# smpurkis/PyTorch-Face-Detection-from-Scratch

Hardware: AMD Instinct MI355X
Metric: train imgs/sec (PoolResnet 480^2, bs=256 per GPU) (higher is better)
Workload: dtype f32 (3x3 convs: bf16x3 split MFMA, fp32 accumulate)

## Files before the change

### pytorch-face-detection-from-scratch_amd/csrc/fdet_conv3x3_ps.hip

```cpp
#include "fdet_conv3x3_x3.h"
#include "fdet_ps.h"
#include "fdet_ldsdma.h"
#include <algorithm>

using namespace fdet;

typedef __attribute__((address_space(3))) void* lds_void_t;
typedef const __attribute__((address_space(1))) void* glb_void_t;
typedef unsigned u32x4 __attribute__((ext_vector_type(4)));

namespace {

#ifndef PS_DBG
#define PS_DBG 0
#endif
constexpr int PSA = 9 * 2 * 64;
constexpr int PS_ROWI = 10;

enum { PSE_FWD_FULL = 0, PSE_DGRAD_ACT = 1, PSE_FWD_POOL = 2, PSE_DGRAD_ADDPOOL = 3 };

struct PsConvArgs {
  const bf16x8* x;
  const bf16x8* a_hi;
  const bf16x8* a_lo;
// ... 22 lines not shown
__device__ __forceinline__ void ps_keep(const f32x16& v) {
#if defined(__HIP_DEVICE_COMPILE__)
  asm volatile("" ::"v"(v));
#endif
}

__device__ __forceinline__ void ps_opaque(unsigned& v) {
#if defined(__HIP_DEVICE_COMPILE__)
  asm("" : "+v"(v));
#endif
}

__device__ __forceinline__ int ps_lane_now() {
  int v = 0;
#if defined(__HIP_DEVICE_COMPILE__)
  asm volatile("v_mbcnt_lo_u32_b32 %0, -1, 0\n\tv_mbcnt_hi_u32_b32 %0, -1, %0" : "=v"(v));
#endif
  return v;
}

__device__ __forceinline__ void ps_acc_read(const f32x16& acc, const int r, float& z) {
#if defined(__HIP_DEVICE_COMPILE__)
  asm("v_accvgpr_read_b32 %0, %1" : "=v"(z) : "a"(acc[r]));
#else
  z = acc[r];
#endif
}

template <int MODE, bool P16>
__device__ __forceinline__ void ps_unit(const f32x16& acc, const int gp, const float (&bza)[4], const float (&bzb)[4],
                                        const u32x2_t (&sg)[2], const float slope, const bool ok, const int ob, const int m,
                                        const int half, const int gstride, const int plane_o_bytes,
                                        const __amdgpu_buffer_rsrc_t yrs) {
  float za[4], zb[4];
#pragma unroll
  for (int i = 0; i < 4; ++i) {
#if defined(__HIP_DEVICE_COMPILE__)
    asm("v_accvgpr_read_b32 %0, %1" : "=v"(za[i]) : "a"(acc[8 * gp + i]));
    asm("v_accvgpr_read_b32 %0, %1" : "=v"(zb[i]) : "a"(acc[8 * gp + 4 + i]));
#else
    za[i] = acc[8 * gp + i]; zb[i] = acc[8 * gp + 4 + i];
#endif
  }
  if (MODE == PSE_FWD_FULL) {
#pragma unroll
    for (int i = 0; i < 4; ++i) {
      const float wa = za[i] + bza[i], wb = zb[i] + bzb[i];
      za[i] = fmaxf(wa, wa * slope);
      zb[i] = fmaxf(wb, wb * slope);
    }
  } else if (MODE == PSE_DGRAD_ACT) {
#pragma unroll
    for (int i = 0; i < 4; ++i) {
      za[i] *= ps_join(sg[0][i >> 1], 0u, i & 1) > 0.f ? 1.f : slope;
      zb[i] *= ps_join(sg[1][i >> 1], 0u, i & 1) > 0.f ? 1.f : slope;
    }
  }
  unsigned ha[2], la[2], hb[2], lb[2];
  if (P16) {
    ps_hi4(za, ha);
    ps_hi4(zb, hb);
  } else {
    ps_split4(za, ha, la);
    ps_split4(zb, hb, lb);
  }
#pragma unroll
  for (int k = 0; k < 2; ++k) {
    auto r1 = __builtin_amdgcn_permlane32_swap(ha[k], hb[k], false, false);
    ha[k] = r1[0]; hb[k] = r1[1];
    if (!P16) {
      auto r2 = __builtin_amdgcn_permlane32_swap(la[k], lb[k], false, false);
      la[k] = r2[0]; lb[k] = r2[1];
    }
  }
  const int G = 4 * m + 2 * gp + half;
  const unsigned off = ok ? (unsigned)(ob + G * gstride) * 16u : 0x80000000u;
  __builtin_amdgcn_raw_buffer_store_b128(u32x4{ha[0], ha[1], hb[0], hb[1]}, yrs, off, 0, 0);
  if (!P16) __builtin_amdgcn_raw_buffer_store_b128(u32x4{la[0], la[1], lb[0], lb[1]}, yrs, off, plane_o_bytes, 0);
}

template <int MODE, int WP, bool P16, bool WG2 = false>
__global__ void __launch_bounds__(256, WG2 ? 2 : 1)
k_conv3x3_ps(const PsConvArgs p) {
  static_assert(!WG2 || MODE == PSE_FWD_POOL, "two workgroups per CU: the pooled forward only (one accumulator set)");
  constexpr bool WOVEN = MODE == PSE_FWD_FULL || MODE == PSE_DGRAD_ACT || MODE == PSE_DGRAD_ADDPOOL;
  extern __shared__ __attribute__((aligned(16))) char smem[];
  bf16x8* const lds = reinterpret_cast<bf16x8*>(smem);
  const int tid = threadIdx.x, lane = tid & 63;
  const int wid = __builtin_amdgcn_readfirstlane(tid >> 6);
  const int l31 = lane & 31, half = lane >> 5;
  constexpr int WPL = WP == 64 ? 6 : 5, R = 512 / WP, PT = (R + 2) * WP + 8, NBI = (R + 2) * WP / 64;
  constexpr int buf_units = 2 * PSA + 4 * PT;
  const int HP = p.HP;
  int qn[4];
#pragma unroll
  for (int n = 0; n < 4; ++n) qn[n] = WP == 64 ? (2 * wid + (n & 1)) * 64 + (n >> 1) * 32 : (4 * wid + n) * 32;
  constexpr bool POOLM = MODE == PSE_FWD_POOL || MODE == PSE_DGRAD_ADDPOOL;
  if (POOLM) {
#pragma unroll
    for (int n = 0; n < 4; ++n) qn[n] = (WP == 64 ? (2 * wid + (n >> 1)) * 64 : (4 * wid + (n >> 1)) * 32) + (n & 1);
  }
  const int lb = POOLM ? (WP == 64 ? 2 * l31 : 2 * l31 + 32 * (l31 >> 4)) : l31;
  int tile = blockIdx.x, tend = p.ntiles, tstep = gridDim.x;
  if ((gridDim.x & 7) == 0) {
    const int grp = blockIdx.x & 7, chunk = (p.ntiles + 7) >> 3;
    tile = grp * chunk + (blockIdx.x >> 3);
    tend = min((grp + 1) * chunk, p.ntiles);
    tstep = gridDim.x >> 3;
    if (tile >= tend) tile = tend = p.ntiles;
  }
  if (tile >= tend) return;

  unsigned ro[PS_ROWI];
#define PS_ROWOFF(T)                                                                               \
  {                                                                                                \
    const int v0_ = (T) * R;                                                                       \
    _Pragma("unroll") for (int i_ = 0; i_ < PS_ROWI; ++i_) {                                       \
      const int u_ = i_ * 64 + lane;                                                               \
      const int vv_ = v0_ - 1 + (u_ >> WPL) + HP;                                                  \
      const int nn_ = (int)__umulhi((unsigned)vv_, p.magic_hp);                                    \
      ro[i_] = (unsigned)(((PS_DBG & 8) ? 1 : nn_) * p.img_i + (vv_ - nn_ * HP) * WP + (u_ & (WP - 1))) * 16u; \
    }                                                                                              \
  }
  const unsigned lds0 = (unsigned)(size_t)(lds_void_t)smem;
  const dma_u32x4 wrs = dma_rsrc((wid >> 1) ? p.a_lo : p.a_hi, (unsigned)p.nch * PSA * 16u);
  const dma_u32x4 xrs = dma_rsrc(p.x - p.img_i, (unsigned)(p.N + 2) * (unsigned)p.img_i * 16u);
  const unsigned wvoff = (unsigned)((wid & 1) * 576 + lane) * 16u;
#define PS_DMA(C, BS)                                                                              \
  if (!(PS_DBG & 4) && !(P16 && wid >= 2)) {                  \
    const unsigned db_ = lds0 + (unsigned)(BS) * (buf_units * 16);                                 \
    const unsigned ad_ = db_ + (unsigned)((wid >> 1) * PSA + (wid & 1) * 576) * 16u;               \
    _Pragma("unroll") for (int k_ = 0; k_ < ((PS_DBG & 16) ? 0 : 9); ++k_)                          \
      dma_piece(ad_ + k_ * 1024, wvoff, wrs, (unsigned)(C) * (PSA * 16) + k_ * 1024);              \
    const unsigned bso_ = (unsigned)((wid >> 1) * p.plane_i + (2 * (C) + (wid & 1)) * HP * WP) * 16u; \
    const unsigned bd_ = db_ + (unsigned)(2 * PSA + wid * PT) * 16u;                               \
    _Pragma("unroll") for (int i_ = 0; i_ < NBI; ++i_) dma_piece(bd_ + i_ * 1024, ro[i_], xrs, bso_); \
  }

  f32x16 accA[2][4], accB[WOVEN ? 2 : 1][WOVEN ? 4 : 1];
  if (WOVEN) {
#pragma unroll
    for (int m = 0; m < 2; ++m)
#pragma unroll
      for (int n = 0; n < 4; ++n)
#pragma unroll
        for (int r = 0; r < 16; ++r) accB[WOVEN ? m : 0][WOVEN ? n : 0][r] = 0.f;
  }

  float bz[2][4][4];
#pragma unroll
  for (int m = 0; m < 2; ++m)
#pragma unroll
    for (int g = 0; g < 4; ++g)
#pragma unroll
      for (int i = 0; i < 4; ++i) bz[m][g][i] = ((MODE == PSE_FWD_FULL || MODE == PSE_FWD_POOL) && !WG2) ? p.bias[32 * m + 8 * g + 4 * half + i] : 0.f;

  const int a_off = half * 64 + l31;
  const int b_off = 2 * PSA + half * PT + lb;
  const int gstride = HP * WP, plane_o_bytes = p.plane_o * 16;
  const __amdgpu_buffer_rsrc_t yrs = __builtin_amdgcn_make_buffer_rsrc(p.y, 0, (int)((size_t)p.N * p.img_o * 16), 0x00020000);

  int ob[4];
  bool okn[4];
#pragma unroll
  for (int n = 0; n < 4; ++n) { ob[n] = 0; okn[n] = false; }
#define PS_GEO(T)                                                                                  \
  {                                                                                                \
    _Pragma("unroll") for (int n_ = 0; n_ < 4; ++n_) {                                             \
// ... 95 lines not shown
    }                                                                                              \
    _Pragma("unroll") for (int n_ = 0; n_ < 4; ++n_) {                                             \
      bh[F][n_] = Bw[qn[n_] + to_];                                                                \
      if (!P16) bl[F][n_] = Bw[2 * PT + qn[n_] + to_];                                             \
    }                                                                                              \
  }
#define PS_BODY(ACC, FIRST, JOB, PREV)                                                             \
  {                                                                                                \
    const bf16x8* buf_ = lds + sb * buf_units;                                                     \
    const bf16x8* Aw = buf_ + a_off;                                                               \
    const bf16x8* Bw = buf_ + b_off;                                                               \
    PS_FRAGS(0, 0)                                                                                 \
    __builtin_amdgcn_sched_barrier(0);                                                             \
    _Pragma("unroll") for (int t = 0; t < 9; ++t) {                                                \
      const int F = t & 1;                                                                         \
      if (t < 8) PS_FRAGS(F ^ 1, t + 1)                                                            \
      if (!(PS_DBG & 2)) {                                                                         \
        _Pragma("unroll") for (int m = 0; m < 2; ++m)                                              \
          _Pragma("unroll") for (int n = 0; n < 4; ++n) {                                          \
            const f32x16 zero_ = {};                                                               \
            if (P16) {                                                                             \
              ACC[m][n] = __builtin_amdgcn_mfma_f32_32x32x16_bf16(ah[F][m], bh[F][n], ((FIRST) && t == 0) ? zero_ : ACC[m][n], 0, 0, 0); \
            } else {                                                                               \
              ACC[m][n] = __builtin_amdgcn_mfma_f32_32x32x16_bf16(ah[F][m], bl[F][n], ((FIRST) && t == 0) ? zero_ : ACC[m][n], 0, 0, 0); \
              ACC[m][n] = __builtin_amdgcn_mfma_f32_32x32x16_bf16(al[F][m], bh[F][n], ACC[m][n], 0, 0, 0); \
              ACC[m][n] = __builtin_amdgcn_mfma_f32_32x32x16_bf16(ah[F][m], bh[F][n], ACC[m][n], 0, 0, 0); \
            }                                                                                      \
          }                                                                                        \
      }                                                                                            \
      if ((JOB) != 0 && t < 8 && !(PS_DBG & 1)) {                                                  \
        if constexpr (MODE == PSE_DGRAD_ADDPOOL) {                                                 \
           \
          _Pragma("unroll") for (int e_ = 0; e_ < 2; ++e_) {                                       \
            const int it_ = ((JOB) - 1) * 16 + 2 * t + e_;                                         \
            const int m_ = it_ >> 4, gp_ = (it_ >> 3) & 1, ab_ = (it_ >> 2) & 1, i_ = it_ & 3;     \
            const int arg_ = (int)((rkp[m_][gp_][ab_] >> (8 * i_ + 4)) & 3u);                      \
            const float gv_ = dgp[m_][gp_][ab_][i_];                                               \
            const int so_ = (32 * m_ + 16 * gp_ + 8 * ab_ + i_) * p.H * p.Wf * 4;                  \
            _Pragma("unroll") for (int r_ = 0; r_ < 2; ++r_) {                                     \
              float z0_, z1_;                                                                      \
              ps_acc_read(PREV[WOVEN ? m_ : 0][WOVEN ? 2 * r_ : 0], 8 * gp_ + 4 * ab_ + i_, z0_);  \
              ps_acc_read(PREV[WOVEN ? m_ : 0][WOVEN ? 2 * r_ + 1 : 0], 8 * gp_ + 4 * ab_ + i_, z1_); \
              z0_ += arg_ == 2 * r_ ? gv_ : 0.f;                                                   \
              z1_ += arg_ == 2 * r_ + 1 ? gv_ : 0.f;                                               \
              __builtin_amdgcn_raw_buffer_store_b64(u32x2_t{__builtin_bit_cast(unsigned, z0_), __builtin_bit_cast(unsigned, z1_)}, prs, sto, \
                                                    so_ + r_ * p.Wf * 4, 0);                       \
            }                                                                                      \
          }                                                                                        \
        } else {                                                                                   \
          const int n_ = ((JOB) - 1) * 2 + (t >> 2), m_ = (t >> 1) & 1, gp_ = t & 1;               \
          ps_unit<MODE, P16>(PREV[WOVEN ? m_ : 0][WOVEN ? n_ : 0], gp_, bz[m_][2 * gp_], bz[m_][2 * gp_ + 1], sgp[n_][m_][gp_], p.slope, okn[n_], ob[n_], m_, \
                        half, gstride, plane_o_bytes, yrs);                                        \
        }                                                                                          \
      }                                                                                            \
       \
       \
      if (P16) {    \
        _Pragma("unroll") for (int i = 0; i < 8; ++i) {                                            \
          __builtin_amdgcn_sched_group_barrier(0x008, 1, 0);                                       \
          if (i < 6) __builtin_amdgcn_sched_group_barrier(0x100, 1, 0);                            \
          if ((JOB) != 0) __builtin_amdgcn_sched_group_barrier(0x002, 6, 0);                       \
          if ((JOB) != 0 && (i >= 7 || (MODE == PSE_DGRAD_ADDPOOL && i >= 4))) __builtin_amdgcn_sched_group_barrier(0x040, 1, 0); \
        }                                                                                          \
      } else {                                                                                     \
      _Pragma("unroll") for (int i = 0; i < 12; ++i) {                                             \
        __builtin_amdgcn_sched_group_barrier(0x008, 1, 0);                                         \
        __builtin_amdgcn_sched_group_barrier(0x100, 1, 0);                                         \
        if ((JOB) != 0) __builtin_amdgcn_sched_group_barrier(0x002, 3, 0);                         \
      }                                                                                            \
      _Pragma("unroll") for (int i = 0; i < 12; ++i) {                                             \
        __builtin_amdgcn_sched_group_barrier(0x008, 1, 0);                                         \
        if ((JOB) != 0) __builtin_amdgcn_sched_group_barrier(0x002, 3, 0);                         \
        if ((JOB) != 0 && (i >= 10 || (MODE == PSE_DGRAD_ADDPOOL && i >= 8))) __builtin_amdgcn_sched_group_barrier(0x040, 1, 0); \
      }                                                                                            \
      }                                                                                            \
    }                                                                                              \
    sb ^= 1;                                                                                       \
  }
  const __amdgpu_buffer_rsrc_t prs = __builtin_amdgcn_make_buffer_rsrc(MODE == PSE_FWD_POOL ? (void*)p.pool_ps : (void*)p.dx_f32, 0,
      MODE == PSE_FWD_POOL ? (int)((size_t)p.N * p.img_p * 16) : (int)((size_t)p.Nimg * 64 * p.H * p.Wf * 4), 0x00020000);
  const __amdgpu_buffer_rsrc_t frs = __builtin_amdgcn_make_buffer_rsrc(p.pool_f32, 0, (int)((size_t)p.Nimg * 64 * p.Hp * p.Wpf * 4), 0x00020000);
  const __amdgpu_buffer_rsrc_t rrs = __builtin_amdgcn_make_buffer_rsrc(p.route_out, 0, (int)((size_t)p.N * 64 * p.Hp * p.Wp), 0x00020000);
  const __amdgpu_buffer_rsrc_t srs = __builtin_amdgcn_make_buffer_rsrc((void*)p.scale, 0, (WG2 && p.scale) ? (int)((size_t)p.Nimg * 64 * 4) : 0, 0x00020000);
  const __amdgpu_buffer_rsrc_t ars = __builtin_amdgcn_make_buffer_rsrc((void*)p.aux, 0, WG2 ? (int)((size_t)p.N * p.img_i * 16) : 0, 0x00020000);
  const __amdgpu_buffer_rsrc_t brs = __builtin_amdgcn_make_buffer_rsrc((void*)p.bias, 0, (WG2 && p.bias) ? 64 * 4 : 0, 0x00020000);
  const int pool_cnt = MODE == PSE_FWD_POOL ? 4 * ((P16 ? 1 : 2) * (p.pool_ps != nullptr) + (p.route_out != nullptr) + 8 * (p.pool_f32 != nullptr)) : 63;
#define PS_WIN(T)                                                                                  \
    const int rb_ = WP == 64 ? 2 * wid : 4 * wid + 2 * (l31 >> 4);                                 \
    const int v_ = (T) * R + rb_;                                                                  \
    const int nn = (int)__umulhi((unsigned)v_, p.magic_hp), y = v_ - nn * HP;                      \
    const int xp = WP == 64 ? l31 : (l31 & 15), yp = y >> 1;                                       \
    const bool okw = nn < p.N && y < p.H && 2 * xp < (nn >= p.last0 ? p.Wlast : p.W);              \
                \
    const int si = p.last0 == 0 ? 0 : (p.Nimg == 1 ? nn : (int)__umulhi((unsigned)nn, p.magic_nimg)); \
    const int ni = nn - si * p.Nimg, xg = si * (p.xo >> 1) + xp;
  float dgp[2][2][2][4];
  unsigned rkp[2][2][2];
  unsigned sto = 0x80000000u;
#pragma unroll
  for (int m = 0; m < 2; ++m)
#pragma unroll
    for (int gp = 0; gp < 2; ++gp)
#pragma unroll
      for (int ab = 0; ab < 2; ++ab) {
        rkp[m][gp][ab] = 0u;
#pragma unroll
        for (int i = 0; i < 4; ++i) dgp[m][gp][ab][i] = 0.f;
      }
#define PS_POOLPREF(T)                                                                             \
  {                                                                                                \
    PS_WIN(T)                                                                                      \
    const int HWp = p.Hp * p.Wpf, HWr = p.Hp * p.Wp;                                               \
    const int pbase = okw ? (ni * 64 * p.Hp + yp) * p.Wpf + xg : 0;                                \
    const int rbase = okw ? (nn * 8 * p.Hp + yp) * p.Wp + xp : 0;                                  \
    _Pragma("unroll") for (int m = 0; m < 2; ++m)                                                  \
      _Pragma("unroll") for (int gp = 0; gp < 2; ++gp)                                             \
        _Pragma("unroll") for (int ab = 0; ab < 2; ++ab) {                                         \
          const int G = 4 * m + 2 * gp + ab;                                                       \
          _Pragma("unroll") for (int i = 0; i < 4; ++i) {                                          \
            const float v_ = p.dout[pbase + (8 * G + 4 * half + i) * HWp];                         \
            dgp[m][gp][ab][i] = okw ? v_ : 0.f;                                                    \
          }                                                                                        \
          rkp[m][gp][ab] = *reinterpret_cast<const unsigned*>(p.route_in + (size_t)(rbase + G * HWr) * 8 + 4 * half); \
        }                                                                                          \
    sto = okw ? (unsigned)(((ni * 64 + 4 * half) * p.H + y) * p.Wf + 2 * xg) * 4u : 0x80000000u;   \
  }
#define PS_EPI_LOADS(M, GP)                                                                        \
  {                                                                                                \
    const size_t ga = (size_t)(4 * (M) + 2 * (GP)) * gstride, gb = ga + (size_t)gstride;           \
    _Pragma("unroll") for (int n = 0; n < 4; ++n) {                                                \
      const u32x2_t* ap = reinterpret_cast<const u32x2_t*>(p.aux + sb0 + (n >> 1) * WP + (n & 1)) + half; \
      sk[M][GP][n][0] = ap[ga * 2];                                                                \
      sk[M][GP][n][1] = P16 ? u32x2_t{0u, 0u} : ap[(ga + p.plane_i) * 2];                          \
      sk[M][GP][n][2] = ap[gb * 2];                                                                \
      sk[M][GP][n][3] = P16 ? u32x2_t{0u, 0u} : ap[(gb + p.plane_i) * 2];                          \
    }                                                                                              \
    _Pragma("unroll") for (int i = 0; i < 4; ++i) {                                                \
      const int ch = 32 * (M) + 16 * (GP) + 4 * half + i;                                          \
      scv[M][GP][0][i] = (p.scale && okw) ? p.scale[ni * 64 + ch] : 1.f;                           \
      scv[M][GP][1][i] = (p.scale && okw) ? p.scale[ni * 64 + ch + 8] : 1.f;                       \
      bzw[M][2 * (GP)][i] = bz[M][2 * (GP)][i];                                                    \
      bzw[M][2 * (GP) + 1][i] = bz[M][2 * (GP) + 1][i];                                            \
    }                                                                                              \
  }
#define PS_EPI_LOADS_G(M, GP, AB)                                                                  \
  {                                                                                                \
    const int g_ = (4 * (M) + 2 * (GP) + (AB)) * gstride * 16;                                     \
    _Pragma("unroll") for (int n = 0; n < 4; ++n) {    \
      const int n_ = ((n >> 1) * WP + (n & 1)) * 16;                                               \
      sk[M][GP][n][2 * (AB)] = __builtin_amdgcn_raw_buffer_load_b64(ars, skoff, g_ + n_, 0);       \
      sk[M][GP][n][2 * (AB) + 1] = P16 ? u32x2_t{0u, 0u} : __builtin_amdgcn_raw_buffer_load_b64(ars, skoff, g_ + p.plane_i * 16 + n_, 0); \
    }                                                                                              \
    _Pragma("unroll") for (int i = 0; i < 4; ++i) {                                                \
      const int ch = 32 * (M) + 16 * (GP) + 8 * (AB) + i;                                          \
      const unsigned sv_ = __builtin_amdgcn_raw_buffer_load_b32(srs, scoff, ch * 4, 0);            \
      scv[M][GP][AB][i] = __uint_as_float((sv_ & scm) | (0x3f800000u & ~scm));    \
      bzw[M][2 * (GP) + (AB)][i] = __uint_as_float(__builtin_amdgcn_raw_buffer_load_b32(brs, (unsigned)halfe * 16u, ch * 4, 0)); \
    }                                                                                              \
  }
#define PS_EPI_ST_F32(M, GP)                                                                       \
  {                                                                                                \
    const unsigned off = okw ? (unsigned)(((ni * 64 + 32 * (M) + 16 * (GP) + 4 * halfe) * p.Hp + yp) * p.Wpf + xg) * 4u : 0x80000000u;\
    _Pragma("unroll") for (int jj = 0; jj < 8; ++jj)                                               \
      __builtin_amdgcn_raw_buffer_store_b32(__builtin_bit_cast(unsigned, pvs[M][GP][jj >> 2][jj & 3]), frs, off,\
                                            (8 * (jj >> 2) + (jj & 3)) * p.Hp * p.Wpf * 4, 0);     \
  }
#define PS_EPI_XCHG(M, GP)                                                                         \
// ... 62 lines not shown
          }                                                                                        \
          _Pragma("unroll") for (int i = 0; i < 4; ++i) {                                          \
            float mx = -INFINITY;                                                                  \
            int arg = 0;                                                                           \
            unsigned bits = 0;                                                                     \
            _Pragma("unroll") for (int n = 0; n < 4; ++n) {                                        \
              float z;                                                                             \
              ps_acc_read(ACC[m][n], 8 * gp + 4 * ab + i, z);                                      \
              const float w_ = z + bzw[m][2 * gp + ab][i];                                         \
              z = fmaxf(w_, w_ * p.slope);                                                         \
              bits |= (z > 0.f ? 1u : 0u) << n;                                                    \
              const float u_ = z * scv[m][gp][ab][i] + ps_join(sk[m][gp][n][2 * ab][i >> 1], sk[m][gp][n][2 * ab + 1][i >> 1], i & 1); \
              if (u_ > mx || u_ != u_) { mx = u_; arg = n; }    \
            }                                                                                      \
            pvs[m][gp][ab][i] = mx;                                                                \
            rt[ab] |= (bits | ((unsigned)arg << 4)) << (8 * i);                                    \
            if (WG2) __builtin_amdgcn_sched_barrier(0);    \
          }                                                                                        \
        }                                                                                          \
        rts[m][gp][0] = rt[0]; rts[m][gp][1] = rt[1];                                              \
        if (WG2) {   \
          if (p.pool_f32) PS_EPI_ST_F32(m, gp)                                                     \
          PS_EPI_XCHG(m, gp)                                                                       \
          if (p.pool_ps) PS_EPI_ST_PS(m, gp)                                                       \
          if (p.route_out) PS_EPI_ST_RT(m, gp)                                                     \
        }                                                                                          \
      }                                                                                            \
    if (!WG2) {                                                                                    \
      if (p.pool_f32) {                                                                            \
        _Pragma("unroll") for (int m = 0; m < 2; ++m)                                              \
          _Pragma("unroll") for (int gp = 0; gp < 2; ++gp) PS_EPI_ST_F32(m, gp)                    \
      }                                                                                            \
      _Pragma("unroll") for (int m = 0; m < 2; ++m)                                                \
        _Pragma("unroll") for (int gp = 0; gp < 2; ++gp) PS_EPI_XCHG(m, gp)                        \
      if (p.pool_ps) {                                                                             \
        _Pragma("unroll") for (int m = 0; m < 2; ++m)                                              \
          _Pragma("unroll") for (int gp = 0; gp < 2; ++gp) PS_EPI_ST_PS(m, gp)                     \
      }                                                                                            \
      if (p.route_out) {                                                                           \
        _Pragma("unroll") for (int m = 0; m < 2; ++m)                                              \
          _Pragma("unroll") for (int gp = 0; gp < 2; ++gp) PS_EPI_ST_RT(m, gp)                     \
      }                                                                                            \
    }                                                                                              \
    }                                                                                              \
  } else {                                                                                         \
    _Pragma("unroll") for (int m = 0; m < 2; ++m)                                                  \
      _Pragma("unroll") for (int n = 0; n < 4; ++n) ps_keep(ACC[m][n]);                            \
  }
#define PS_EPI_ADDPOOL(ACC, T)                                                                     \
  if (!(PS_DBG & 1)) {                                                                             \
    PS_WIN(T)                                                                                      \
    float dg[2][2][2][4];                                                                          \
    unsigned rk[2][2][2];                                                                          \
    const int HWp = p.Hp * p.Wpf;                                                                  \
    const int pbase = okw ? (ni * 64 * p.Hp + yp) * p.Wpf + xg : 0;                                \
    _Pragma("unroll") for (int m = 0; m < 2; ++m)                                                  \
      _Pragma("unroll") for (int gp = 0; gp < 2; ++gp)                                             \
        _Pragma("unroll") for (int ab = 0; ab < 2; ++ab) {                                         \
          const int G = 4 * m + 2 * gp + ab;                                                       \
          _Pragma("unroll") for (int i = 0; i < 4; ++i) dg[m][gp][ab][i] = okw ? p.dout[pbase + (8 * G + 4 * half + i) * HWp] : 0.f; \
          rk[m][gp][ab] = okw ? *reinterpret_cast<const unsigned*>(p.route_in + (size_t)(((nn * 8 + G) * p.Hp + yp) * p.Wp + xp) * 8 + 4 * half) : 0u; \
        }                                                                                          \
    _Pragma("unroll") for (int m = 0; m < 2; ++m)                                                  \
      _Pragma("unroll") for (int gp = 0; gp < 2; ++gp)                                             \
        _Pragma("unroll") for (int ab = 0; ab < 2; ++ab)                                           \
          _Pragma("unroll") for (int i = 0; i < 4; ++i) {                                          \
            const int ch = 32 * m + 16 * gp + 8 * ab + 4 * half + i;                               \
            const int arg = (int)((rk[m][gp][ab] >> (8 * i + 4)) & 3u);                            \
            const float gv = dg[m][gp][ab][i];                                                     \
            _Pragma("unroll") for (int r = 0; r < 2; ++r) {                                        \
              float z0, z1;                                                                        \
              ps_acc_read(ACC[m][2 * r], 8 * gp + 4 * ab + i, z0);                                 \
              ps_acc_read(ACC[m][2 * r + 1], 8 * gp + 4 * ab + i, z1);                             \
              z0 += arg == 2 * r ? gv : 0.f;                                                       \
              z1 += arg == 2 * r + 1 ? gv : 0.f;                                                   \
              const unsigned off = okw ? (unsigned)(((ni * 64 + ch) * p.H + y + r) * p.Wf + 2 * xg) * 4u : 0x80000000u; \
              __builtin_amdgcn_raw_buffer_store_b64(u32x2_t{__builtin_bit_cast(unsigned, z0), __builtin_bit_cast(unsigned, z1)}, prs, off, 0, 0); \
            }                                                                                      \
          }                                                                                        \
  } else {                                                                                         \
    _Pragma("unroll") for (int m = 0; m < 2; ++m)                                                  \
      _Pragma("unroll") for (int n = 0; n < 4; ++n) ps_keep(ACC[m][n]);                            \
  }
#define PS_EPILOGUE(ACC)                                                                           \
  if constexpr (MODE == PSE_FWD_POOL) { PS_EPI_FWD_POOL(ACC, etile) }                              \
  else if constexpr (MODE == PSE_DGRAD_ADDPOOL) { PS_EPI_ADDPOOL(ACC, etile) }                     \
  else if (!(PS_DBG & 1)) {                                                                        \
    if (MODE == PSE_DGRAD_ACT) PS_SIGNS()                                                          \
    _Pragma("unroll") for (int n = 0; n < 4; ++n)                                                  \
      _Pragma("unroll") for (int m = 0; m < 2; ++m)                                                \
        _Pragma("unroll") for (int gp = 0; gp < 2; ++gp)                                           \
          ps_unit<MODE, P16>(ACC[m][n], gp, bz[m][2 * gp], bz[m][2 * gp + 1], sgp[n][m][gp], p.slope,  \
                        okn[n], ob[n], m, half, gstride, plane_o_bytes, yrs);                      \
  } else {                                                                                         \
    _Pragma("unroll") for (int m = 0; m < 2; ++m)                                                  \
      _Pragma("unroll") for (int n = 0; n < 4; ++n) ps_keep(ACC[m][n]);                            \
  }
#define PS_TILE(ACC, PREV)                                                                         \
  {                                                                                                \
    PS_OPEN()                                                                                      \
    PS_NEXT(0)                                                                                     \
    PS_BODY(ACC, 1, (WOVEN ? 1 : 0), PREV)                                                         \
    young = (WOVEN && !(PS_DBG & 1)) ? (MODE == PSE_DGRAD_ADDPOOL ? 32 : (P16 ? 8 : 16)) : 0;      \
    PS_OPEN()                                                                                      \
    PS_NEXT(1)                                                                                     \
    PS_BODY(ACC, 0, (WOVEN ? 2 : 0), PREV)                                                         \
    for (int c = 2; c < p.nch; ++c) {                                                              \
      PS_OPEN()                                                                                    \
      PS_NEXT(c)                                                                                   \
      PS_BODY(ACC, 0, 0, PREV)                                                                     \
      young = 0;                                                                                   \
    }                                                                                              \
    PS_GEO(tile)                                                                                   \
    etile = tile;                                                                                  \
    if (WOVEN && MODE == PSE_DGRAD_ACT && !(PS_DBG & 1)) {                                         \
      PS_SIGNS()                                                                                   \
      young += 32;                                                                                 \
    }                                                                                              \
    if constexpr (MODE == PSE_DGRAD_ADDPOOL) {                                                     \
      if (!(PS_DBG & 1)) {                                                                         \
        PS_POOLPREF(tile)                                                                          \
        young = min(young + 40, 63);                                                               \
      }                                                                                            \
    }                                                                                              \
    if (!WOVEN) {                                                                                  \
      PS_EPILOGUE(ACC)                                                                             \
      young = (PS_DBG & 1) ? 0 : (POOLM ? pool_cnt : 32);                                          \
    }                                                                                              \
  }

#define PS_TILE2(ACC)                                                                              \
  {                                                                                                \
    PS_OPEN()                                                                                      \
    PS_BODY2(ACC, 1)                                                                               \
    for (int c = 1; c < p.nch; ++c) {                                                              \
      __builtin_amdgcn_s_barrier();                                                                \
      { const int lane = ps_lane_now(); PS_ROWOFF(tile) }   \
      PS_DMA(c, 0)                                                                                 \
      __builtin_amdgcn_sched_barrier(0);                                                           \
      asm volatile("s_waitcnt vmcnt(0)" ::: "memory");                                             \
      __builtin_amdgcn_s_barrier();                                                                \
      PS_BODY2(ACC, 0)                                                                             \
    }                                                                                              \
    __builtin_amdgcn_s_barrier();                                                                  \
    if (tile + tstep < tend) {                                                                     \
      { const int lane = ps_lane_now(); PS_ROWOFF(tile + tstep) }                                  \
      PS_DMA(0, 0)                                                                                 \
    }                                                                                              \
    __builtin_amdgcn_sched_barrier(0);                                                             \
    etile = tile;                                                                                  \
    PS_EPILOGUE(ACC)                                                                               \
    young = (PS_DBG & 1) ? 0 : pool_cnt;                                                           \
  }

  int etile = tile;
  PS_ROWOFF(tile)
  PS_DMA(0, 0)
  if constexpr (WG2) {
    for (; tile < tend; tile += tstep) PS_TILE2(accA)
  } else if (WOVEN) {
    for (;;) {
      PS_TILE(accA, accB)
      tile += tstep;
      if (tile >= tend) { PS_EPILOGUE(accA) break; }
      PS_TILE(accB, accA)
      tile += tstep;
      if (tile >= tend) { PS_EPILOGUE(accB) break; }
    }
  } else {
    for (; tile < tend; tile += tstep) PS_TILE(accA, accA)
  }
#undef PS_TILE2
#undef PS_TILE
#undef PS_EPILOGUE
#undef PS_EPI_ADDPOOL
#undef PS_EPI_FWD_POOL
#undef PS_EPI_ST_RT
#undef PS_EPI_ST_PS
#undef PS_EPI_XCHG
#undef PS_EPI_ST_F32
#undef PS_EPI_LOADS_G
#undef PS_EPI_LOADS
#undef PS_BODY2
#undef PS_FRAG_B
#undef PS_FRAG_A
#undef PS_POOLPREF
#undef PS_WIN
#undef PS_WAITN
#undef PS_BODY
#undef PS_FRAGS
#undef PS_NEXT
#undef PS_OPEN
#undef PS_GEO
#undef PS_SIGNS
#undef PS_DMA
#undef PS_ROWOFF
}

#ifndef PS_TU
#define PS_TU (-1)
#endif
#define PS_CAT_(a, b) a##b
#define PS_CAT(a, b) PS_CAT_(a, b)
#define PS_TU_NAME PS_CAT(fdet_ps_launch_, PS_TU)
template <int MODE, int WP, bool P16, bool WG2 = false>
int launch_ps(const PsConvArgs& p, size_t lds, int grid, hipStream_t st) {
  static bool attr_set = false;
  constexpr int lds_max = (WG2 ? 1 : 2) * (2 * PSA + 4 * 648) * 16;
  if (!attr_set) {
    if ((int)lds > lds_max || hipFuncSetAttribute((const void*)k_conv3x3_ps<MODE, WP, P16, WG2>, hipFuncAttributeMaxDynamicSharedMemorySize, lds_max) != hipSuccess) {
      (void)hipGetLastError();
      return fail(FDET_ELAUNCH, "conv3x3_ps: cannot reserve %zu bytes of LDS", lds);
    }
    attr_set = true;
  }
  hipLaunchKernelGGL((k_conv3x3_ps<MODE, WP, P16, WG2>), dim3(grid), dim3(256), lds, st, p);
  return check_launch("fdet_conv3x3_ps");
}

}
#define PS_DECL_LAUNCH(N) extern "C" int fdet_ps_launch_##N(const void* args, size_t lds, int grid, void* stream);
PS_DECL_LAUNCH(0) PS_DECL_LAUNCH(1) PS_DECL_LAUNCH(2) PS_DECL_LAUNCH(3) PS_DECL_LAUNCH(4) PS_DECL_LAUNCH(5) PS_DECL_LAUNCH(6) PS_DECL_LAUNCH(7)
PS_DECL_LAUNCH(8) PS_DECL_LAUNCH(9) PS_DECL_LAUNCH(10) PS_DECL_LAUNCH(11) PS_DECL_LAUNCH(12) PS_DECL_LAUNCH(13) PS_DECL_LAUNCH(14) PS_DECL_LAUNCH(15)
PS_DECL_LAUNCH(wg2_4) PS_DECL_LAUNCH(wg2_5)
#if PS_TU >= 0
extern "C" int PS_TU_NAME(const void* args, size_t lds, int grid, void* stream) {
  return launch_ps<(PS_TU & 7) / 2, (PS_TU & 1) ? 64 : 32, (PS_TU >= 8)>(*reinterpret_cast<const PsConvArgs*>(args), lds, grid, (hipStream_t)stream);
}
#endif
#if PS_TU == 4 || PS_TU == 5
extern "C" int PS_CAT(fdet_ps_launch_wg2_, PS_TU)(const void* args, size_t lds, int grid, void* stream) {
  return launch_ps<PSE_FWD_POOL, (PS_TU & 1) ? 64 : 32, false, true>(*reinterpret_cast<const PsConvArgs*>(args), lds, grid, (hipStream_t)stream);
}
#endif
namespace {
#if PS_TU == -1
typedef int (*ps_launch_fn)(const void*, size_t, int, void*);
const ps_launch_fn PS_LAUNCHERS[16] = {fdet_ps_launch_0, fdet_ps_launch_1, fdet_ps_launch_2, fdet_ps_launch_3,
                                       fdet_ps_launch_4, fdet_ps_launch_5, fdet_ps_launch_6, fdet_ps_launch_7,
                                       fdet_ps_launch_8, fdet_ps_launch_9, fdet_ps_launch_10, fdet_ps_launch_11,
                                       fdet_ps_launch_12, fdet_ps_launch_13, fdet_ps_launch_14, fdet_ps_launch_15};
constexpr bool PS_WG2_DEFAULT_64 = true, PS_WG2_DEFAULT_32 = true;
struct PsPoolIO {
  const float* scale = nullptr; void* pool_ps = nullptr; float* pool_f32 = nullptr; unsigned char* route_out = nullptr;
  const float* dout = nullptr; const unsigned char* route_in = nullptr; float* dx_f32 = nullptr;
};

const char* ps_conv_refusal(int pooled, int N, int Cin, int Cout, int H, int W) {
  PsGeo gi, go, gp;
  PsStrips sp, spo;
  if (!(Cout == 64 && Cin % 16 == 0 && Cin >= 32)) return "Cout must be 64 and Cin a multiple of 16, at least 32";
  if (!(ps_geo_strips(N, Cin, H, W, gi, sp) && ps_geo_strips(N, Cout, H, W, go, spo) && gi.WP >= 32 && sp.Ws + 2 <= gi.WP))
    return "unsupported map (W + 2 <= 32 or 64 slots, or an even width in strips)";
  if (!((size_t)(gi.N + 2) * gi.img * 16 < ((size_t)1 << 32) && (size_t)(go.N + 2) * go.img * 16 < ((size_t)1 << 32)))
    return "tensor too large for the 32-bit byte offsets of the DMA descriptors";
  if (pooled) {
    if ((H & 1) || (W & 1) || Cin != 64) return "pooled block: even map and 64 channels required";
    if ((size_t)N * 64 * H * W * 4 >= ((size_t)1 << 31)) return "pooled block: tensor too large for 32-bit offsets";
    if (pooled == 2 && sp.S != 1) return "a strip map writes its pooled output as fp32 NCHW (pool_f32)";
    if (pooled == 2 && !ps_geo(gi.N, 64, H / 2, W / 2, gp)) return "the pooled map has no PS layout";
  }
  if ((long)gi.N * gi.HP + gi.HP >= (1 << 20)) return "too many rows";
  return nullptr;
}

int run_ps(int mode, const void* x, const void* wpk, const float* bias, const void* aux, void* y, const PsPoolIO& io, int N,
           int Cin, int Cout, int H, int W, float slope, hipStream_t st, bool p16 = false) {
  PsGeo gi, gp;
  PsStrips sp;
  const bool pooled = mode == PSE_FWD_POOL || mode == PSE_DGRAD_ADDPOOL;
  FDET_REQUIRE(x && wpk && (y || pooled), "conv3x3_ps: null pointer");
  const int pool_mode = !pooled ? 0 : (mode == PSE_FWD_POOL && io.pool_ps ? 2 : 1);
  if (const char* why = ps_conv_refusal(pool_mode, N, Cin, Cout, H, W))
    return fail(FDET_EINVAL, "conv3x3_ps: %s (N=%d Cin=%d Cout=%d H=%d W=%d)", why, N, Cin, Cout, H, W);
  ps_geo_strips(N, Cin, H, W, gi, sp);
  const int Nimg = N, Wfull = W;
  N = gi.N; W = sp.Ws;
  FDET_REQUIRE(slope >= 0.f && slope <= 1.f, "conv3x3_ps: slope must be in [0, 1]");
  PsConvArgs p;
  p.x = reinterpret_cast<const bf16x8*>(x);
  const size_t units = (size_t)(Cin / 16) * PSA;
  p.a_hi = reinterpret_cast<const bf16x8*>(wpk);
  p.a_lo = p.a_hi + units;
  p.bias = bias;
  p.y = reinterpret_cast<bf16x8*>(y);
  p.aux = reinterpret_cast<const bf16x8*>(aux);
  p.scale = io.scale; p.pool_ps = reinterpret_cast<bf16x8*>(io.pool_ps); p.pool_f32 = io.pool_f32; p.route_out = io.route_out;
  p.dout = io.dout; p.route_in = io.route_in; p.dx_f32 = io.dx_f32;
  p.Hp = H / 2; p.Wp = W / 2; p.HPp = p.WPp = p.plane_p = p.img_p = 0;
  p.Nimg = Nimg; p.last0 = sp.S > 1 ? (sp.S - 1) * Nimg : 0; p.Wlast = sp.Wlast; p.Wf = Wfull; p.Wpf = Wfull / 2; p.xo = sp.Ws;
  p.magic_nimg = Nimg > 1 ? magic_of(Nimg) : 0u;
  PsGeo go;
  PsStrips spo;
  ps_geo_strips(Nimg, Cout, H, Wfull, go, spo);
  if (pool_mode == 2) {
    ps_geo(N, 64, H / 2, W / 2, gp);
    p.HPp = gp.HP; p.WPp = gp.WP; p.plane_p = gp.plane; p.img_p = gp.img;
  }
  p.N = N; p.H = H; p.W = W; p.HP = gi.HP;
  p.nch = Cin / 16;
  const int R = 512 / gi.WP, PT = (R + 2) * gi.WP + 8;
  const long vr = (long)N * gi.HP;
  p.ntiles = (int)((vr + R - 1) / R);
  p.plane_i = gi.plane; p.img_i = gi.img; p.plane_o = go.plane; p.img_o = go.img;
  p.magic_hp = magic_of(gi.HP);
  p.slope = slope;
  size_t lds = (size_t)2 * (2 * PSA + 4 * PT) * 16;
  int grid = std::min(p.ntiles, num_cus());
  const bool w64 = gi.WP == 64;
  static const int wg2_env = [] { const char* e = getenv("FDET_PS_POOL_WG2"); return (e && (e[0] == '0' || e[0] == '1') && !e[1]) ? e[0] - '0' : -1; }();
  bool wg2 = mode == PSE_FWD_POOL && !p16 && (wg2_env >= 0 ? wg2_env == 1 : (w64 ? PS_WG2_DEFAULT_64 : PS_WG2_DEFAULT_32));
  if (wg2 && 2 * (lds / 2) > (size_t)160 * 1024) wg2 = false;
  if (wg2) {
    lds /= 2;
    grid = std::min(p.ntiles, 2 * num_cus());
  }
  switch (mode) {
    case PSE_FWD_FULL:
      FDET_REQUIRE(bias, "conv3x3_ps_fwd: bias is required");
      break;
    case PSE_DGRAD_ACT:
      FDET_REQUIRE(aux, "conv3x3_ps_dgrad_act: the activation is required");
      break;
    case PSE_FWD_POOL:
      FDET_REQUIRE(bias && aux && (io.pool_ps || io.pool_f32), "conv3x3_ps_fwd_pool: bias, skip and an output are required");
      break;
    default:
      FDET_REQUIRE(io.dout && io.route_in && io.dx_f32, "conv3x3_ps_dgrad_unpool: dout, route and dx are required");
      break;
  }
  if (wg2) return (w64 ? fdet_ps_launch_wg2_5 : fdet_ps_launch_wg2_4)(&p, lds, grid, (void*)st);
  return PS_LAUNCHERS[(p16 ? 8 : 0) + 2 * mode + (w64 ? 1 : 0)](&p, lds, grid, (void*)st);
}
#endif

}

#if PS_TU == -1
extern "C" int fdet_conv3x3_ps_ok(int N, int Cin, int Cout, int H, int W, int pooled) {
  return ps_conv_refusal(pooled, N, Cin, Cout, H, W) == nullptr;
}

extern "C" int fdet_conv3x3_ps_fwd(const void* x_ps, const void* wpk, const float* bias, void* y_ps, int N, int Cin,
                                   int Cout, int H, int W, float slope, void* stream) {
  return run_ps(PSE_FWD_FULL, x_ps, wpk, bias, nullptr, y_ps, PsPoolIO{}, N, Cin, Cout, H, W, slope, (hipStream_t)stream);
}

extern "C" int fdet_conv3x3_ps_dgrad_act(const void* dz_ps, const void* wpk, const void* act_ps, void* dx_ps, int N,
                                         int Cin, int Cout, int H, int W, float slope, void* stream) {
  return run_ps(PSE_DGRAD_ACT, dz_ps, wpk, nullptr, act_ps, dx_ps, PsPoolIO{}, N, Cout, Cin, H, W, slope, (hipStream_t)stream);
}

extern "C" int fdet_conv3x3_ps_fwd_pool(const void* x_ps, const void* wpk, const float* bias, const void* skip_ps,
                                        const float* drop_scale, void* pool_ps, float* pool_f32, unsigned char* route8,
                                        int N, int Cin, int Cout, int H, int W, float slope, void* stream) {
  PsPoolIO io;
  io.scale = drop_scale; io.pool_ps = pool_ps; io.pool_f32 = pool_f32; io.route_out = route8;
  return run_ps(PSE_FWD_POOL, x_ps, wpk, bias, skip_ps, nullptr, io, N, Cin, Cout, H, W, slope, (hipStream_t)stream);
}

extern "C" int fdet_conv3x3_ps_dgrad_unpool(const void* dz_ps, const void* wpk, const float* dout_pooled,
                                            const unsigned char* route8, float* dx, int N, int Cin, int Cout, int H, int W,
                                            float slope, void* stream) {
  PsPoolIO io;
  io.dout = dout_pooled; io.route_in = route8; io.dx_f32 = dx;
  return run_ps(PSE_DGRAD_ADDPOOL, dz_ps, wpk, nullptr, nullptr, nullptr, io, N, Cout, Cin, H, W, slope, (hipStream_t)stream);
}

extern "C" int fdet_conv3x3_ps_fwd_p16(const void* x_ps, const void* wpk, const float* bias, void* y_ps, int N, int Cin,
                                       int Cout, int H, int W, float slope, void* stream) {
  return run_ps(PSE_FWD_FULL, x_ps, wpk, bias, nullptr, y_ps, PsPoolIO{}, N, Cin, Cout, H, W, slope, (hipStream_t)stream, true);
}
extern "C" int fdet_conv3x3_ps_dgrad_act_p16(const void* dz_ps, const void* wpk, const void* act_ps, void* dx_ps, int N,
                                             int Cin, int Cout, int H, int W, float slope, void* stream) {
  return run_ps(PSE_DGRAD_ACT, dz_ps, wpk, nullptr, act_ps, dx_ps, PsPoolIO{}, N, Cout, Cin, H, W, slope, (hipStream_t)stream, true);
}
extern "C" int fdet_conv3x3_ps_fwd_pool_p16(const void* x_ps, const void* wpk, const float* bias, const void* skip_ps,
                                            const float* drop_scale, void* pool_ps, float* pool_f32, unsigned char* route8,
                                            int N, int Cin, int Cout, int H, int W, float slope, void* stream) {
  PsPoolIO io;
  io.scale = drop_scale; io.pool_ps = pool_ps; io.pool_f32 = pool_f32; io.route_out = route8;
  return run_ps(PSE_FWD_POOL, x_ps, wpk, bias, skip_ps, nullptr, io, N, Cin, Cout, H, W, slope, (hipStream_t)stream, true);
}
extern "C" int fdet_conv3x3_ps_dgrad_unpool_p16(const void* dz_ps, const void* wpk, const float* dout_pooled,
                                                const unsigned char* route8, float* dx, int N, int Cin, int Cout, int H, int W,
                                                float slope, void* stream) {
  PsPoolIO io;
  io.dout = dout_pooled; io.route_in = route8; io.dx_f32 = dx;
  return run_ps(PSE_DGRAD_ADDPOOL, dz_ps, wpk, nullptr, nullptr, nullptr, io, N, Cout, Cin, H, W, slope, (hipStream_t)stream, true);
}

#endif
```

Before: 93480.

## Extend two-workgroups-per-CU mode to full forward and dgrad 3x3 conv kernels

Generalizes the WG2 (two workgroups per CU, half LDS each) variant from the pooled forward to all four bf16x3 conv modes. It adds new single-accumulator-set epilogues for plain forward/dgrad-act and for dgrad-addpool, which software-pipeline their global loads. It also adds per-mode env overrides and enables WG2 by default for the 32-wide maps of those modes. The aim is latency hiding through higher occupancy in place of intra-kernel weaving, at the cost of non-woven epilogues and a smaller LDS budget per workgroup.

```diff
diff --git a/pytorch-face-detection-from-scratch_amd/csrc/fdet_conv3x3_ps.hip b/pytorch-face-detection-from-scratch_amd/csrc/fdet_conv3x3_ps.hip
--- a/pytorch-face-detection-from-scratch_amd/csrc/fdet_conv3x3_ps.hip
+++ b/pytorch-face-detection-from-scratch_amd/csrc/fdet_conv3x3_ps.hip
@@ -128,8 +128,8 @@
 template <int MODE, int WP, bool P16, bool WG2 = false>
 __global__ void __launch_bounds__(256, WG2 ? 2 : 1)
 k_conv3x3_ps(const PsConvArgs p) {
-  static_assert(!WG2 || MODE == PSE_FWD_POOL, "two workgroups per CU: the pooled forward only (one accumulator set)");
-  constexpr bool WOVEN = MODE == PSE_FWD_FULL || MODE == PSE_DGRAD_ACT || MODE == PSE_DGRAD_ADDPOOL;
+  static_assert(!WG2 || !P16, "two workgroups per CU: the bf16x3 instantiations only");
+  constexpr bool WOVEN = !WG2 && (MODE == PSE_FWD_FULL || MODE == PSE_DGRAD_ACT || MODE == PSE_DGRAD_ADDPOOL);
   extern __shared__ __attribute__((aligned(16))) char smem[];
   bf16x8* const lds = reinterpret_cast<bf16x8*>(smem);
   const int tid = threadIdx.x, lane = tid & 63;
@@ -391,7 +391,9 @@
   const __amdgpu_buffer_rsrc_t frs = __builtin_amdgcn_make_buffer_rsrc(p.pool_f32, 0, (int)((size_t)p.Nimg * 64 * p.Hp * p.Wpf * 4), 0x00020000);
   const __amdgpu_buffer_rsrc_t rrs = __builtin_amdgcn_make_buffer_rsrc(p.route_out, 0, (int)((size_t)p.N * 64 * p.Hp * p.Wp), 0x00020000);
   const __amdgpu_buffer_rsrc_t srs = __builtin_amdgcn_make_buffer_rsrc((void*)p.scale, 0, (WG2 && p.scale) ? (int)((size_t)p.Nimg * 64 * 4) : 0, 0x00020000);
-  const __amdgpu_buffer_rsrc_t ars = __builtin_amdgcn_make_buffer_rsrc((void*)p.aux, 0, WG2 ? (int)((size_t)p.N * p.img_i * 16) : 0, 0x00020000);
+  const __amdgpu_buffer_rsrc_t ars = __builtin_amdgcn_make_buffer_rsrc((void*)p.aux, 0, (WG2 && p.aux) ? (int)((size_t)p.N * (MODE == PSE_DGRAD_ACT ? p.img_o : p.img_i) * 16) : 0, 0x00020000);
+  const __amdgpu_buffer_rsrc_t drs = __builtin_amdgcn_make_buffer_rsrc((void*)p.dout, 0, (WG2 && MODE == PSE_DGRAD_ADDPOOL) ? (int)((size_t)p.Nimg * 64 * p.Hp * p.Wpf * 4) : 0, 0x00020000);
+  const __amdgpu_buffer_rsrc_t irs = __builtin_amdgcn_make_buffer_rsrc((void*)p.route_in, 0, (WG2 && MODE == PSE_DGRAD_ADDPOOL) ? (int)((size_t)p.N * 64 * p.Hp * p.Wp) : 0, 0x00020000);
   const __amdgpu_buffer_rsrc_t brs = __builtin_amdgcn_make_buffer_rsrc((void*)p.bias, 0, (WG2 && p.bias) ? 64 * 4 : 0, 0x00020000);
   const int pool_cnt = MODE == PSE_FWD_POOL ? 4 * ((P16 ? 1 : 2) * (p.pool_ps != nullptr) + (p.route_out != nullptr) + 8 * (p.pool_f32 != nullptr)) : 63;
 #define PS_WIN(T)                                                                                  \
@@ -620,8 +622,101 @@
     _Pragma("unroll") for (int m = 0; m < 2; ++m)                                                  \
       _Pragma("unroll") for (int n = 0; n < 4; ++n) ps_keep(ACC[m][n]);                            \
   }
+#define PS_EPI_PLAIN2(ACC, T)                                                                      \
+  if (!(PS_DBG & 1)) {                                                                             \
+    const int ln_ = ps_lane_now();                                                                 \
+    const int l31 = ln_ & 31, half = ln_ >> 5;                                                     \
+    PS_GEO(T)                                                                                      \
+    unsigned sgo[4];                                                                               \
+    _Pragma("unroll") for (int n = 0; n < 4; ++n) {                                                \
+      unsigned km_ = okn[n] ? 0xffffffffu : 0u;                                                    \
+      ps_opaque(km_);                                                                              \
+      sgo[n] = (((unsigned)ob[n] * 16u + (unsigned)half * 8u) & km_) | (0x80000000u & ~km_);       \
+    }                                                                                              \
+    u32x2_t sg[2][2] = {};                                                                         \
+    float bzu[2][4] = {};                                                                          \
+    if (MODE == PSE_DGRAD_ACT) {                                                                   \
+      sg[0][0] = __builtin_amdgcn_raw_buffer_load_b64(ars, sgo[0], 0, 0);                          \
+      sg[0][1] = __builtin_amdgcn_raw_buffer_load_b64(ars, sgo[0], gstride * 16, 0);               \
+    }                                                                                              \
+    _Pragma("unroll") for (int m = 0; m < 2; ++m)                                                  \
+      _Pragma("unroll") for (int gp = 0; gp < 2; ++gp) {                                           \
+        if (MODE == PSE_FWD_FULL) {                                                                \
+          _Pragma("unroll") for (int i = 0; i < 4; ++i) {                                          \
+            bzu[0][i] = __uint_as_float(__builtin_amdgcn_raw_buffer_load_b32(brs, (unsigned)half * 16u, (32 * m + 16 * gp + i) * 4, 0)); \
+            bzu[1][i] = __uint_as_float(__builtin_amdgcn_raw_buffer_load_b32(brs, (unsigned)half * 16u, (32 * m + 16 * gp + 8 + i) * 4, 0)); \
+          }                                                                                        \
+        }                                                                                          \
+        _Pragma("unroll") for (int n = 0; n < 4; ++n) {                                            \
+          const int u_ = (2 * m + gp) * 4 + n;                                                     \
+          if (MODE == PSE_DGRAD_ACT) {                                                             \
+            __builtin_amdgcn_sched_barrier(0);                                                     \
+            if (u_ + 1 < 16) {                                                                     \
+              const int n1_ = (u_ + 1) & 3, g1_ = 2 * ((u_ + 1) >> 2);    \
+              sg[(u_ + 1) & 1][0] = __builtin_amdgcn_raw_buffer_load_b64(ars, sgo[n1_], g1_ * gstride * 16, 0); \
+              sg[(u_ + 1) & 1][1] = __builtin_amdgcn_raw_buffer_load_b64(ars, sgo[n1_], (g1_ + 1) * gstride * 16, 0); \
+            }                                                                                      \
+          }                                                                                        \
+          ps_unit<MODE, P16>(ACC[m][n], gp, bzu[0], bzu[1], sg[u_ & 1], p.slope, okn[n], ob[n], m, half, gstride, plane_o_bytes, yrs); \
+           \
+           \
+           \
+          __builtin_amdgcn_sched_barrier(0);                                                       \
+          asm volatile("s_nop 3");                                                                 \
+          __builtin_amdgcn_sched_barrier(0);                                                       \
+        }                                                                                          \
+      }                                                                                            \
+  } else {                                                                                         \
+    _Pragma("unroll") for (int m = 0; m < 2; ++m)                                                  \
+      _Pragma("unroll") for (int n = 0; n < 4; ++n) ps_keep(ACC[m][n]);                            \
+  }
+#define PS_ADDPOOL2_LOADS(G, S)                                                                    \
+  {                                                                                                \
+    _Pragma("unroll") for (int i = 0; i < 4; ++i)                                                  \
+      dg[S][i] = __uint_as_float(__builtin_amdgcn_raw_buffer_load_b32(drs, dvo, (8 * (G) + i) * HWp * 4, 0)); \
+    rk[S] = __builtin_amdgcn_raw_buffer_load_b32(irs, rvo, (G) * HWr * 8, 0);                      \
+  }
+#define PS_EPI_ADDPOOL2(ACC, T)                                                                    \
+  if (!(PS_DBG & 1)) {                                                                             \
+    const int ln_ = ps_lane_now();                                                                 \
+    const int l31 = ln_ & 31, half = ln_ >> 5;                                                     \
+    PS_WIN(T)                                                                                      \
+    const int HWp = p.Hp * p.Wpf, HWr = p.Hp * p.Wp;                                               \
+    unsigned km = okw ? 0xffffffffu : 0u;                                                          \
+    ps_opaque(km);                                                                                 \
+    const unsigned oor = 0x80000000u & ~km;                                                        \
+    const unsigned dvo = ((unsigned)((ni * 64 * p.Hp + yp) * p.Wpf + xg + 4 * half * HWp) * 4u & km) | oor; \
+    const unsigned rvo = ((unsigned)(((nn * 8 * p.Hp + yp) * p.Wp + xp) * 8 + 4 * half) & km) | oor; \
+    const unsigned sto2 = ((unsigned)(((ni * 64 + 4 * half) * p.H + y) * p.Wf + 2 * xg) * 4u & km) | oor; \
+    float dg[2][4];                                                                                \
+    unsigned rk[2];                                                                                \
+    PS_ADDPOOL2_LOADS(0, 0)                                                                        \
+    _Pragma("unroll") for (int G = 0; G < 8; ++G) {                                                \
+      const int m = G >> 2, gp = (G >> 1) & 1, ab = G & 1;                                         \
+      __builtin_amdgcn_sched_barrier(0);                                                           \
+      if (G < 7) PS_ADDPOOL2_LOADS(G + 1, (G + 1) & 1)                                             \
+      _Pragma("unroll") for (int i = 0; i < 4; ++i) {                                              \
+        const int arg = (int)((rk[G & 1] >> (8 * i + 4)) & 3u);                                    \
+        const float gv = dg[G & 1][i];                                                             \
+        _Pragma("unroll") for (int r = 0; r < 2; ++r) {                                            \
+          float z0, z1;                                                                            \
+          ps_acc_read(ACC[m][2 * r], 8 * gp + 4 * ab + i, z0);                                     \
+          ps_acc_read(ACC[m][2 * r + 1], 8 * gp + 4 * ab + i, z1);                                 \
+          z0 += arg == 2 * r ? gv : 0.f;                                                           \
+          z1 += arg == 2 * r + 1 ? gv : 0.f;                                                       \
+          __builtin_amdgcn_raw_buffer_store_b64(u32x2_t{__builtin_bit_cast(unsigned, z0), __builtin_bit_cast(unsigned, z1)}, prs, sto2, \
+                                                ((8 * G + i) * p.H + r) * p.Wf * 4, 0);            \
+        }                                                                                          \
+      }                                                                                            \
+    }                                                                                              \
+  } else {                                                                                         \
+    _Pragma("unroll") for (int m = 0; m < 2; ++m)                                                  \
+      _Pragma("unroll") for (int n = 0; n < 4; ++n) ps_keep(ACC[m][n]);                            \
+  }
 #define PS_EPILOGUE(ACC)                                                                           \
   if constexpr (MODE == PSE_FWD_POOL) { PS_EPI_FWD_POOL(ACC, etile) }                              \
+  else if constexpr (WG2 && MODE == PSE_DGRAD_ADDPOOL) { PS_EPI_ADDPOOL2(ACC, etile) }             \
+  else if constexpr (WG2) { PS_EPI_PLAIN2(ACC, etile) }                                            \
   else if constexpr (MODE == PSE_DGRAD_ADDPOOL) { PS_EPI_ADDPOOL(ACC, etile) }                     \
   else if (!(PS_DBG & 1)) {                                                                        \
     if (MODE == PSE_DGRAD_ACT) PS_SIGNS()                                                          \
@@ -688,7 +783,7 @@
     __builtin_amdgcn_sched_barrier(0);                                                             \
     etile = tile;                                                                                  \
     PS_EPILOGUE(ACC)                                                                               \
-    young = (PS_DBG & 1) ? 0 : pool_cnt;                                                           \
+    young = (PS_DBG & 1) ? 0 : (POOLM ? pool_cnt : 32);                                            \
   }
 
   int etile = tile;
@@ -711,6 +806,9 @@
 #undef PS_TILE2
 #undef PS_TILE
 #undef PS_EPILOGUE
+#undef PS_EPI_ADDPOOL2
+#undef PS_ADDPOOL2_LOADS
+#undef PS_EPI_PLAIN2
 #undef PS_EPI_ADDPOOL
 #undef PS_EPI_FWD_POOL
 #undef PS_EPI_ST_RT
@@ -760,15 +858,16 @@
 #define PS_DECL_LAUNCH(N) extern "C" int fdet_ps_launch_##N(const void* args, size_t lds, int grid, void* stream);
 PS_DECL_LAUNCH(0) PS_DECL_LAUNCH(1) PS_DECL_LAUNCH(2) PS_DECL_LAUNCH(3) PS_DECL_LAUNCH(4) PS_DECL_LAUNCH(5) PS_DECL_LAUNCH(6) PS_DECL_LAUNCH(7)
 PS_DECL_LAUNCH(8) PS_DECL_LAUNCH(9) PS_DECL_LAUNCH(10) PS_DECL_LAUNCH(11) PS_DECL_LAUNCH(12) PS_DECL_LAUNCH(13) PS_DECL_LAUNCH(14) PS_DECL_LAUNCH(15)
-PS_DECL_LAUNCH(wg2_4) PS_DECL_LAUNCH(wg2_5)
+PS_DECL_LAUNCH(wg2_0) PS_DECL_LAUNCH(wg2_1) PS_DECL_LAUNCH(wg2_2) PS_DECL_LAUNCH(wg2_3) PS_DECL_LAUNCH(wg2_4) PS_DECL_LAUNCH(wg2_5)
+PS_DECL_LAUNCH(wg2_6) PS_DECL_LAUNCH(wg2_7)
 #if PS_TU >= 0
 extern "C" int PS_TU_NAME(const void* args, size_t lds, int grid, void* stream) {
   return launch_ps<(PS_TU & 7) / 2, (PS_TU & 1) ? 64 : 32, (PS_TU >= 8)>(*reinterpret_cast<const PsConvArgs*>(args), lds, grid, (hipStream_t)stream);
 }
 #endif
-#if PS_TU == 4 || PS_TU == 5
+#if PS_TU >= 0 && PS_TU < 8
 extern "C" int PS_CAT(fdet_ps_launch_wg2_, PS_TU)(const void* args, size_t lds, int grid, void* stream) {
-  return launch_ps<PSE_FWD_POOL, (PS_TU & 1) ? 64 : 32, false, true>(*reinterpret_cast<const PsConvArgs*>(args), lds, grid, (hipStream_t)stream);
+  return launch_ps<PS_TU / 2, (PS_TU & 1) ? 64 : 32, false, true>(*reinterpret_cast<const PsConvArgs*>(args), lds, grid, (hipStream_t)stream);
 }
 #endif
 namespace {
@@ -778,7 +877,19 @@
                                        fdet_ps_launch_4, fdet_ps_launch_5, fdet_ps_launch_6, fdet_ps_launch_7,
                                        fdet_ps_launch_8, fdet_ps_launch_9, fdet_ps_launch_10, fdet_ps_launch_11,
                                        fdet_ps_launch_12, fdet_ps_launch_13, fdet_ps_launch_14, fdet_ps_launch_15};
+inline int env_flag01(const char* name) {
+  const char* e = getenv(name);
+  return (e && (e[0] == '0' || e[0] == '1') && !e[1]) ? e[0] - '0' : -1;
+}
 constexpr bool PS_WG2_DEFAULT_64 = true, PS_WG2_DEFAULT_32 = true;
+constexpr bool PS_WG2_DEFAULT[4][2] = {{true, false}, {true, false}, {PS_WG2_DEFAULT_32, PS_WG2_DEFAULT_64}, {true, false}};
+const ps_launch_fn PS_WG2_LAUNCHERS[8] = {fdet_ps_launch_wg2_0, fdet_ps_launch_wg2_1, fdet_ps_launch_wg2_2, fdet_ps_launch_wg2_3,
+                                          fdet_ps_launch_wg2_4, fdet_ps_launch_wg2_5, fdet_ps_launch_wg2_6, fdet_ps_launch_wg2_7};
+int ps_wg2_env(int mode) {
+  static const int env[4] = {env_flag01("FDET_PS_FWD_WG2"), env_flag01("FDET_PS_DGRAD_ACT_WG2"), env_flag01("FDET_PS_POOL_WG2"),
+                             env_flag01("FDET_PS_DGRAD_UNPOOL_WG2")};
+  return env[mode];
+}
 struct PsPoolIO {
   const float* scale = nullptr; void* pool_ps = nullptr; float* pool_f32 = nullptr; unsigned char* route_out = nullptr;
   const float* dout = nullptr; const unsigned char* route_in = nullptr; float* dx_f32 = nullptr;
@@ -846,8 +957,8 @@
   size_t lds = (size_t)2 * (2 * PSA + 4 * PT) * 16;
   int grid = std::min(p.ntiles, num_cus());
   const bool w64 = gi.WP == 64;
-  static const int wg2_env = [] { const char* e = getenv("FDET_PS_POOL_WG2"); return (e && (e[0] == '0' || e[0] == '1') && !e[1]) ? e[0] - '0' : -1; }();
-  bool wg2 = mode == PSE_FWD_POOL && !p16 && (wg2_env >= 0 ? wg2_env == 1 : (w64 ? PS_WG2_DEFAULT_64 : PS_WG2_DEFAULT_32));
+  const int wg2_env = ps_wg2_env(mode);
+  bool wg2 = !p16 && (wg2_env >= 0 ? wg2_env == 1 : PS_WG2_DEFAULT[mode][w64 ? 1 : 0]);
   if (wg2 && 2 * (lds / 2) > (size_t)160 * 1024) wg2 = false;
   if (wg2) {
     lds /= 2;
@@ -867,7 +978,7 @@
       FDET_REQUIRE(io.dout && io.route_in && io.dx_f32, "conv3x3_ps_dgrad_unpool: dout, route and dx are required");
       break;
   }
-  if (wg2) return (w64 ? fdet_ps_launch_wg2_5 : fdet_ps_launch_wg2_4)(&p, lds, grid, (void*)st);
+  if (wg2) return PS_WG2_LAUNCHERS[2 * mode + (w64 ? 1 : 0)](&p, lds, grid, (void*)st);
   return PS_LAUNCHERS[(p16 ? 8 : 0) + 2 * mode + (w64 ? 1 : 0)](&p, lds, grid, (void*)st);
 }
 #endif
```

Result: no change. 93920, median of 6 (+0.5%).
